# Sota0726/weather-Unet

Measured on AMD Instinct MI355X. Metric: images/sec 256x256 cUNet fwd+bwd, higher is better.
Workload: dtype bf16; 1 GPU; cUNet 256x256 bf16 B=32/GPU, training step: fwd + bwd (dgrad+wgrad) + grad all-reduce + fused Adam; dropout p=0.3 on; random-init weights, 5-class one-hot, loss mean|G(x,c)-x|; global_batch=32, parallelism=dp1

## Files before the change

scratch/stamp_wgrad.py:

```python


def main():
    import sys, os
    sys.path.insert(0, os.path.join(os.path.dirname(__file__), '..', 'weather-unet_amd'))
    import torch
    from wu import _lib, kernels as K
    dev = torch.device('cuda:0'); B = 32
    NWAVES = int(sys.argv[1]) if len(sys.argv) > 1 else 8
    _lib.call('wu_set_option', 2, 1 if NWAVES == 8 else 2)
    dbg = torch.zeros(256 * 8 * 8, dtype=torch.int64, device=dev)
    for name, ci, co, s in [('d1.2', 64, 64, 256), ('d2.2', 128, 128, 128), ('d4.2', 512, 512, 32), ('u1.0', 192, 64, 256), ('u3.0', 768, 256, 64)]:
        x = (torch.rand((B, s, s, ci), device=dev) * 2 - 1).to(torch.bfloat16).permute(0, 3, 1, 2)
        gy = (torch.rand((B, s, s, co), device=dev) * 2 - 1).to(torch.bfloat16).permute(0, 3, 1, 2)
        dw = torch.empty((co, ci, 3, 3), device=dev); db = torch.empty((co,), device=dev)
        for _ in range(20): K.conv3x3_wgrad(x, gy, dw, db)
        torch.cuda.synchronize()
        _lib.call('wu_set_debug_buffer', dbg.data_ptr()); dbg.zero_()
        e0, e1 = torch.cuda.Event(enable_timing=True), torch.cuda.Event(enable_timing=True)
        e0.record(); K.conv3x3_wgrad(x, gy, dw, db); e1.record(); torch.cuda.synchronize()
        _lib.call('wu_set_debug_buffer', None)
        d = dbg.view(256, 8, 8).double().cpu()[:, :NWAVES]
        d = d[d[:, 0, 6] > 0]
        tiles = d[:, 0, 6].mean().item()
        clk = (d[:, 0, 2] / d[:, 0, 3]).median().item() * 0.1
        w, c, tot, bar = d[:, :, 0].mean().item(), d[:, :, 1].mean().item(), d[:, :, 2].mean().item(), d[:, :, 4].mean().item()
        print(f"{name}: wgrad+reduce {e0.elapsed_time(e1)*1e3:.0f} us, tiles/WG {tiles:.1f}; per tile: dma wait {w/tiles:.0f}, barrier {bar/tiles:.0f}, compute {c/tiles:.0f} (ideal 4608); main loop total/tile {tot/tiles:.0f}; in-kernel clock {clk:.2f} GHz")


if __name__ == "__main__":
    main()
```

weather-unet_amd/csrc/conv3x3_wgrad.hip:

```cpp
#include <type_traits>
#include <utility>

#include "wu_common.h"
#include "wgrad_internal.h"

namespace {

template <typename F, int... I> __device__ __forceinline__ void wgrad_static_for_impl(F&& f, std::integer_sequence<int, I...>) {
    (f(std::integral_constant<int, I>{}), ...);
}
template <int N, typename F> __device__ __forceinline__ void wgrad_static_for(F&& f) { wgrad_static_for_impl(f, std::make_integer_sequence<int, N>{}); }

struct WgradArgs {
    const void* x; const void* dy; const void* y;
    float* slab;
    float* bslab;
    int ldx, lddy, ldy;
    int N, H, W, Ho, Wo, Cin, Cout;
    int act;
    int tw_log2, tiles_x, tiles_y, ntiles;
    int splits, co_blocks, ci_blocks;
    int halo_w, halo_h, halo_pix;
};

// ... 275 lines not shown
                const int hp = ry * STRIDE * a.halo_w + rx * STRIDE;
#pragma unroll
                for (int tap = 0; tap < 9; ++tap) {
                    const int kh = tap / 3, kw = tap % 3;
                    const float bv = *(const float*)(x_lds + lds_off<T>(hp + kh * a.halo_w + kw, 0, (32 * wn + l31) * 4));
                    acc[tap] = __builtin_amdgcn_mfma_f32_32x32x2f32(av, bv, acc[tap], 0, 0, 0);
                }
            }
        }
        __syncthreads();
    }

    {
        const int l31 = lane & 31, lh = lane >> 5;
        float* sl = a.slab + (size_t)split * a.Cin;
        const size_t rs = (size_t)a.splits * a.Cin;
#pragma unroll
        for (int tap = 0; tap < 9; ++tap)
#pragma unroll
            for (int i = 0; i < 16; ++i) {
                const int co = cob * 64 + 32 * wm + (i & 3) + 8 * (i >> 2) + 4 * lh;
                const int ci = cib * 64 + 32 * wn + l31;
                sl[((size_t)tap * a.Cout + co) * rs + ci] = acc[tap][i];
            }
    }
    if (cib == 0 && a.bslab) {
        float* red = (float*)smem;
        red[tid] = bsum;
        __syncthreads();
        if (tid < 64) a.bslab[(size_t)split * a.Cout + cob * 64 + tid] = red[tid] + red[tid + 64] + red[tid + 128] + red[tid + 192];
    }
}

__global__ __launch_bounds__(256) __attribute__((amdgpu_num_vgpr(32))) void wgrad_reduce_kernel(
    const float* __restrict__ slab, const float* __restrict__ bslab, float* __restrict__ dw, float* __restrict__ dbias,
    int splits, int Cout, int Cin, int accumulate, int wpr) {
    const int lane = threadIdx.x & 63;
    const int wid = blockIdx.x * 4 + __builtin_amdgcn_readfirstlane((int)(threadIdx.x >> 6));
    const int row = wid / wpr, part = wid - row * wpr;
    if (row >= Cout * 9) return;
    const int co = row / 9, t = row - co * 9;
    const int c4n = (Cin >> 2) / wpr, c4lo = part * c4n;
    int TX = 64;
    while (TX > c4n) TX >>= 1;
    const int G = 64 / TX;
    const int tx = lane & (TX - 1), g = lane / TX;
    const float* base = slab + ((size_t)t * Cout + co) * splits * Cin;
    for (int c4b = 0; c4b < c4n; c4b += TX) {
        const int c4 = c4b + tx;
        const bool valid = c4 < c4n;
        unsigned off = (unsigned)(g * Cin + (c4lo + (valid ? c4 : 0)) * 4);
        const unsigned step = (unsigned)(G * Cin);
        float4 sacc = make_float4(0.f, 0.f, 0.f, 0.f);
        int k = g;
        for (; k + G < splits; k += 2 * G, off += 2 * step) {
            const float4 v0 = *(const float4*)(base + off);
            const float4 v1 = *(const float4*)(base + off + step);
            sacc.x += v0.x; sacc.y += v0.y; sacc.z += v0.z; sacc.w += v0.w;
            sacc.x += v1.x; sacc.y += v1.y; sacc.z += v1.z; sacc.w += v1.w;
        }
        if (k < splits) {
            const float4 v0 = *(const float4*)(base + off);
            sacc.x += v0.x; sacc.y += v0.y; sacc.z += v0.z; sacc.w += v0.w;
        }
        for (int m = TX; m < 64; m <<= 1) {
            sacc.x += __shfl_xor(sacc.x, m); sacc.y += __shfl_xor(sacc.y, m);
            sacc.z += __shfl_xor(sacc.z, m); sacc.w += __shfl_xor(sacc.w, m);
        }
        if (g == 0 && valid) {
            float* o = dw + ((size_t)co * Cin + (c4lo + c4) * 4) * 9 + t;
            if (accumulate) { o[0] += sacc.x; o[9] += sacc.y; o[18] += sacc.z; o[27] += sacc.w; }
            else { o[0] = sacc.x; o[9] = sacc.y; o[18] = sacc.z; o[27] = sacc.w; }
        }
    }
    if (dbias && t == 0 && part == 0) {
        float b = 0.f;
        for (int k = lane; k < splits; k += 64) b += bslab[(size_t)k * Cout + co];
        for (int m = 1; m < 64; m <<= 1) b += __shfl_xor(b, m);
        if (lane == 0) dbias[co] = accumulate ? dbias[co] + b : b;
    }
}

void launch_wgrad_reduce(const float* slab, const float* bslab, float* dw, float* dbias, int splits, int Cout, int Cin, int accumulate, hipStream_t s) {
    int wpr = 1;
    while (wpr < 8 && (long long)splits * (Cin >> 2) > 64LL * 16 * wpr && ((Cin >> 2) % (2 * wpr)) == 0) wpr <<= 1;
    hipLaunchKernelGGL(wgrad_reduce_kernel, dim3(cdiv(Cout * 9 * wpr, 4)), dim3(256), 0, s, slab, bslab, dw, dbias, splits, Cout, Cin, accumulate, wpr);
}

struct WPlan { int P, twl, tiles_x, tiles_y, ntiles, splits, halo_w, halo_h; size_t lds, ws; };

WPlan wgrad_plan(int N, int H, int W, int Cin, int Cout, int stride, int dtype) {
    WPlan p;
    const bool bf = dtype == WU_BF16;
    p.P = bf ? (stride == 1 ? 256 : 128) : (stride == 1 ? 128 : 64);
    const int Ho = (H - 1) / stride + 1, Wo = (W - 1) / stride + 1;
    int twl = 5;
    while (twl > 2 && (1 << (twl - 1)) >= Wo) --twl;
    p.twl = twl;
    const int TW = 1 << twl, TH = p.P >> twl;
    p.tiles_x = cdiv(Wo, TW); p.tiles_y = cdiv(Ho, TH);
    p.ntiles = N * p.tiles_x * p.tiles_y;
    const int blocks = (Cout / 64) * (Cin / 64);
    int splits = cdiv(512, blocks);
    if (splits > p.ntiles) splits = p.ntiles;
    if (splits < 1) splits = 1;
    p.splits = splits;
    p.halo_w = (TW - 1) * stride + 3; p.halo_h = (TH - 1) * stride + 3;
    const int rb = bf ? 128 : 256;
    p.lds = (size_t)(p.P + p.halo_w * p.halo_h) * rb;
    p.ws = ((size_t)splits * 9 * Cout * Cin + (size_t)splits * Cout) * sizeof(float);
    return p;
}

template <typename T, int STRIDE, int P>
void launch_wgrad(const WgradArgs& a, size_t lds, int grid, hipStream_t s) {
    auto kern = conv3x3_wgrad_kernel<T, STRIDE, P>;
    static thread_local bool attr_set = false;
    if (!attr_set) {
        (void)hipFuncSetAttribute((const void*)kern, hipFuncAttributeMaxDynamicSharedMemorySize, 160 * 1024);
// ... 71 lines not shown
```

weather-unet_amd/csrc/conv3x3_wgrad_v2.hip:

```cpp
#include <type_traits>
#include <utility>

#include "wu_common.h"
#include "wgrad_internal.h"

namespace {


struct C {
    static constexpr int P = 256, TH = 8;
    static constexpr int DY_ROW = 128, DY_SLOTS = 8;
    static constexpr int HALO_W = 34, HALO_H = TH + 2, HALO_PIX = HALO_W * HALO_H;
    static constexpr int DY_BYTES = P * DY_ROW;
    static constexpr int DY_PIECES = DY_BYTES / 1024;
    static constexpr int X_PIECES = 48;
    static constexpr int X_BYTES = X_PIECES * 1024;
    static constexpr int BUF = DY_BYTES + X_BYTES;
};

template <int NW_> struct CW {
    static constexpr int NW = NW_;
    static constexpr int NDY = C::DY_PIECES / NW;
    static constexpr int NX = C::X_PIECES / NW;
    static constexpr int PARS = NW == 8 ? 1 : 2;
    static constexpr int NG = 8 * PARS;
};

struct W2Args {
    const bf16_t* x; const bf16_t* dy;
    float* slab; float* bslab;
    unsigned long long* dbg;
    int ldx, lddy;
    int N, H, W, Cin, Cout;
    int tiles_x, tiles_y, ntiles, tiles_per_split, splits, co_blocks, ci_blocks;
    int dma_interleave;
};

__device__ __forceinline__ void dma_wait_all() { asm volatile("s_waitcnt vmcnt(0)" ::: "memory"); }
__device__ __forceinline__ uint4 tr_frag(const char* p0) {
    const s16x4_t a = __builtin_amdgcn_ds_read_tr16_b64_v4i16((s16x4_t __attribute__((address_space(3)))*)p0);
    const s16x4_t b = __builtin_amdgcn_ds_read_tr16_b64_v4i16((s16x4_t __attribute__((address_space(3)))*)(p0 + 4 * 128));
    return make_uint4(((const uint32_t*)&a)[0], ((const uint32_t*)&a)[1], ((const uint32_t*)&b)[0], ((const uint32_t*)&b)[1]);
}
__device__ __forceinline__ void mma(f32x16_t& acc, const uint4& a, const uint4& b) {
    acc = __builtin_amdgcn_mfma_f32_32x32x16_bf16(__builtin_bit_cast(bf16x8_t, a), __builtin_bit_cast(bf16x8_t, b), acc, 0, 0, 0);
}

template <typename F, int... I> __device__ __forceinline__ void static_for_impl(F&& f, std::integer_sequence<int, I...>) {
    (f(std::integral_constant<int, I>{}), ...);
}
template <int N, typename F> __device__ __forceinline__ void static_for(F&& f) { static_for_impl(f, std::make_integer_sequence<int, N>{}); }

template <int HF> __device__ __forceinline__ constexpr int tap_of(int i) { return i == 4 ? 4 : (HF ? 5 + i : i); }

template <int HF, int PARS, typename Issue>
__device__ __forceinline__ void compute_tile(const char* lds, const int (&a_lane)[2], const int (&b_lane)[3], f32x16_t (&acc)[9], Issue&& issue) {
    constexpr int NG = 8 * PARS, NS = 5 * NG;
    auto goff_a = [](int g) { return 32 * (g / PARS) * C::DY_ROW + (g % PARS) * 16 * C::DY_ROW; };
    auto goff_b = [](int g) { return (g / PARS) * C::HALO_W * 128 + (g % PARS) * 16 * 128; };
    auto load_a = [&](int g, int m) __attribute__((always_inline)) { return tr_frag(lds + a_lane[m] + goff_a(g)); };
    auto load_b = [&](int s_) __attribute__((always_inline)) {
        const int g = s_ / 5, i = s_ % 5;
        const int tap = tap_of<HF>(i), kh = tap / 3, kw = tap % 3;
        return tr_frag(lds + b_lane[kw] + goff_b(g) + (kh * C::HALO_W + kw) * 128);
    };
    constexpr int LA = PARS == 1 ? 2 : 5;
    uint4 af[2][2], bf[LA + 1];
    af[0][0] = load_a(0, 0);
// ... 7 lines not shown
        if (PARS == 1) {
            if (i == 0) issue(g);
            if (s_ + LA < NS) bf[(s_ + LA) % (LA + 1)] = load_b(s_ + LA);
            if (g + 1 < NG && i == 1) af[(g + 1) & 1][0] = load_a(g + 1, 0);
            if (g + 1 < NG && i == 2) af[(g + 1) & 1][1] = load_a(g + 1, 1);
            __builtin_amdgcn_sched_barrier(0);
            if constexpr (i < 4) {
                mma(acc[2 * i], af[g & 1][0], b);
                mma(acc[2 * i + 1], af[g & 1][1], b);
            } else {
                mma(acc[8], af[g & 1][HF], b);
            }
            __builtin_amdgcn_sched_barrier(0);
        } else {
            mma(acc[i < 4 ? 2 * i : 8], af[g & 1][i < 4 ? 0 : HF], b);
            if (s_ + LA < NS) bf[(s_ + LA) % (LA + 1)] = load_b(s_ + LA);
            __builtin_amdgcn_sched_barrier(0);
            if constexpr (i < 4) mma(acc[2 * i + 1], af[g & 1][1], b);
            if (g + 1 < NG && i == 1) af[(g + 1) & 1][0] = load_a(g + 1, 0);
            if (g + 1 < NG && i == 2) af[(g + 1) & 1][1] = load_a(g + 1, 1);
            if (i == 0) issue(g);
            __builtin_amdgcn_sched_barrier(0);
        }
    });
}

template <int NW>
__global__ __launch_bounds__(NW * 64) void conv3x3_wgrad_v2_kernel(const W2Args a) {
    using Q = CW<NW>;
    extern __shared__ __attribute__((aligned(16))) char smem[];
    const int tid = threadIdx.x, lane = tid & 63;
    const int wave = __builtin_amdgcn_readfirstlane(tid >> 6);
    const int wci = wave & 1, hf = (wave >> 1) & 1, par = NW == 8 ? wave >> 2 : 0;

    int bid = xcd_remap(blockIdx.x, gridDim.x);
    const int blocks = a.co_blocks * a.ci_blocks;
    const int blk = bid % blocks, split = bid / blocks;
    const int cib = blk % a.ci_blocks, cob = blk / a.ci_blocks;
    const int t_begin = split * a.tiles_per_split;
    const int t_end = min(a.ntiles, t_begin + a.tiles_per_split);

    unsigned dy_off[Q::NDY];
#pragma unroll
    for (int j = 0; j < Q::NDY; ++j) {
        const int i = (NW * j + wave) * 64 + lane;
        const int r = i / C::DY_SLOTS, sl = i % C::DY_SLOTS;
        const int s = sl ^ (((r >> 1) & 1) << 2);
        dy_off[j] = (unsigned)((((r >> 5) * a.W + (r & 31)) * a.lddy + s * 8) * 2);
    }
    unsigned x_off[Q::NX], x_flag[Q::NX];
#pragma unroll
    for (int j = 0; j < Q::NX; ++j) {
        const int i = (NW * j + wave) * 64 + lane;
        const int p = i >> 3, sl = i & 7;
        const int hy = p / C::HALO_W, hx = p - hy * C::HALO_W;
        const int s = sl ^ (((hx >> 1) & 1) << 2);
        x_off[j] = p < C::HALO_PIX ? (unsigned)(((hy * a.W + hx) * a.ldx + s * 8) * 2) : kWuOOB;
        x_flag[j] = (hy == 0 ? 1u : 0u) | (hx == 0 ? 2u : 0u) | (hx == C::HALO_W - 1 ? 4u : 0u);
    }

    const unsigned smem_base = (unsigned)(uintptr_t)(__attribute__((address_space(3))) char*)smem;
    const unsigned dy_img_bytes = (unsigned)((size_t)a.H * a.W * a.lddy * 2);
    const unsigned x_img_bytes = (unsigned)((((size_t)a.H * a.W + a.W) * a.ldx + 64) * 2);
    wu_rsrc_t rs_dy = wu_make_rsrc(a.dy, 0), rs_x = rs_dy;
    unsigned so_dy = 0, so_x = 0, border_f = 0;
    int f_tx = 0, f_ty = 0, f_n = 0;
    {
        int tt = t_begin;
        f_tx = tt % a.tiles_x; tt /= a.tiles_x;
        f_ty = tt % a.tiles_y;
        f_n = tt / a.tiles_y;
    }
    auto set_fetch_tile = [&](bool step) __attribute__((always_inline)) {
        if (step) {
            ++f_tx;
            if (f_tx == a.tiles_x) { f_tx = 0; ++f_ty; }
            if (f_ty == a.tiles_y) { f_ty = 0; ++f_n; }
        }
        const int tx = f_tx, ty = f_ty, n = f_n;
        const int oh0 = ty * C::TH, ow0 = tx * 32;
        rs_dy = wu_make_rsrc(a.dy + (size_t)n * a.H * a.W * a.lddy + cob * 64, dy_img_bytes);
        so_dy = (unsigned)__builtin_amdgcn_readfirstlane((oh0 * a.W + ow0) * a.lddy * 2);
        rs_x = wu_make_rsrc(a.x + ((long long)n * a.H * a.W - (a.W + 1)) * a.ldx + cib * 64, x_img_bytes);
        so_x = (unsigned)__builtin_amdgcn_readfirstlane((oh0 * a.W + ow0) * a.ldx * 2);
        border_f = (unsigned)__builtin_amdgcn_readfirstlane((int)((oh0 == 0 ? 1u : 0u) | (ow0 == 0 ? 2u : 0u) | (ow0 + 32 >= a.W ? 4u : 0u)));
    };
    auto issue_piece = [&](int j, int buf) __attribute__((always_inline)) {
        const unsigned lds = smem_base + buf * C::BUF;
        if (j < Q::NDY) {
            wu_dma16b(dy_off[j], rs_dy, so_dy, __builtin_amdgcn_readfirstlane(lds + (NW * j + wave) * 1024));
        } else {
            const int jj = j - Q::NDY;
            const unsigned vo = (x_flag[jj] & border_f) ? kWuOOB : x_off[jj];
            wu_dma16b(vo, rs_x, so_x, __builtin_amdgcn_readfirstlane(lds + C::DY_BYTES + (NW * jj + wave) * 1024));
        }
    };

    const int g16 = lane >> 4, i16 = lane & 15, q = i16 >> 2, pp = i16 & 3, h = g16 >> 1;
    const int r_lane = 16 * par + 8 * h + q;
    int a_lane[2];
#pragma unroll
    for (int m = 0; m < 2; ++m) {
        const int cb = (32 * m + 16 * (g16 & 1) + 4 * pp) * 2;
        a_lane[m] = r_lane * C::DY_ROW + (cb ^ (((q >> 1) & 1) << 6));
    }
    int b_lane[3];
#pragma unroll
    for (int kw = 0; kw < 3; ++kw) {
        const int cb = (32 * wci + 16 * (g16 & 1) + 4 * pp) * 2;
        b_lane[kw] = C::DY_BYTES + r_lane * 128 + (cb ^ ((((q + kw) >> 1) & 1) << 6));
    }

    f32x16_t acc[9];
#pragma unroll
    for (int t = 0; t < 9; ++t)
#pragma unroll
        for (int i = 0; i < 16; ++i) acc[t][i] = 0.f;
    float bs[8];
#pragma unroll
    for (int e = 0; e < 8; ++e) bs[e] = 0.f;
    const bool do_bias = (cib == 0) && (a.bslab != nullptr);

    unsigned long long t_wait = 0, t_bar = 0, t_comp = 0, t_mark = 0, t_k0 = 0, t_r0 = 0;
#define WU_STAMP(v) do { if (a.dbg) { const unsigned long long t_ = __builtin_readcyclecounter(); v += t_ - t_mark; t_mark = t_; } } while (0)
    if (a.dbg) { t_mark = t_k0 = __builtin_readcyclecounter(); t_r0 = __builtin_amdgcn_s_memrealtime(); }
    auto tile_loop = [&](auto hf_tag) __attribute__((always_inline)) {
        constexpr int HF = decltype(hf_tag)::value;
        if (t_begin < t_end) {
            set_fetch_tile(false);
#pragma unroll
            for (int j = 0; j < Q::NDY + Q::NX; ++j) issue_piece(j, 0);
        }
        for (int tile = t_begin; tile < t_end; ++tile) {
            const int buf = (tile - t_begin) & 1;
            dma_wait_all();
            WU_STAMP(t_wait);
            __syncthreads();
            WU_STAMP(t_bar);
            const bool more = tile + 1 < t_end;
            if (more) set_fetch_tile(true);
            if (more && !a.dma_interleave) {
#pragma unroll
                for (int j = 0; j < Q::NDY + Q::NX; ++j) issue_piece(j, buf ^ 1);
            }
            const char* lds = smem + buf * C::BUF;
            if (do_bias) {
                const int c8 = tid & 7;
#pragma unroll
                for (int r = tid >> 3; r < C::P; r += NW * 8) {
                    const uint4 v = *(const uint4*)(lds + r * C::DY_ROW + ((c8 ^ (((r >> 1) & 1) << 2)) << 4));
                    float f[8];
                    unpack16<bf16_t>(v, f);
#pragma unroll
                    for (int e = 0; e < 8; ++e) bs[e] += f[e];
                }
            }
            compute_tile<HF, Q::PARS>(lds, a_lane, b_lane, acc, [&](int g) __attribute__((always_inline)) {
                if (more && a.dma_interleave && 2 * g < Q::NDY + Q::NX) {
                    issue_piece(2 * g, buf ^ 1);
                    issue_piece(2 * g + 1, buf ^ 1);
                }
            });
            WU_STAMP(t_comp);
        }
    };
    if (hf == 0) tile_loop(std::integral_constant<int, 0>{});
    else tile_loop(std::integral_constant<int, 1>{});
    if (a.dbg && lane == 0) {
        unsigned long long* d = a.dbg + ((size_t)blockIdx.x * 8 + wave) * 8;
        d[0] = t_wait; d[1] = t_comp; d[2] = __builtin_readcyclecounter() - t_k0; d[3] = __builtin_amdgcn_s_memrealtime() - t_r0;
        d[4] = t_bar; d[5] = 0; d[6] = (unsigned long long)(t_end - t_begin); d[7] = 0;
    }
#undef WU_STAMP
    __syncthreads();

    if (NW == 8) {
        float* red = (float*)smem + (size_t)(wave & 3) * 144 * 64;
        if (par == 1) {
#pragma unroll
            for (int t = 0; t < 9; ++t)
#pragma unroll
                for (int i = 0; i < 16; ++i) red[(t * 16 + i) * 64 + lane] = acc[t][i];
        }
        __syncthreads();
        if (par == 0) {
#pragma unroll
            for (int t = 0; t < 9; ++t)
#pragma unroll
                for (int i = 0; i < 16; ++i) acc[t][i] += red[(t * 16 + i) * 64 + lane];
        }
        __syncthreads();
    }

    if (par == 0) {
        const int l31 = lane & 31, lh = lane >> 5;
        float* sl = a.slab + (size_t)split * a.Cin;
        const size_t rs = (size_t)a.splits * a.Cin;
        const int ci = cib * 64 + 32 * wci + l31;
#pragma unroll
        for (int t = 0; t < 9; ++t) {
            const int tap = t == 8 ? 4 : (hf ? 5 + (t >> 1) : (t >> 1));
            const int m = t == 8 ? hf : (t & 1);
#pragma unroll
            for (int i = 0; i < 16; ++i) {
                const int co = cob * 64 + 32 * m + (i & 3) + 8 * (i >> 2) + 4 * lh;
                sl[((size_t)tap * a.Cout + co) * rs + ci] = acc[t][i];
            }
        }
    }
    if (do_bias) {
        float* red = (float*)smem;
#pragma unroll
        for (int e = 0; e < 8; ++e) red[tid * 8 + e] = bs[e];
        __syncthreads();
        if (tid < 64) {
            float s = 0.f;
            for (int j = 0; j < NW * 8; ++j) s += red[(j * 8 + (tid >> 3)) * 8 + (tid & 7)];
            a.bslab[(size_t)split * a.Cout + cob * 64 + tid] = s;
        }
    }
}

}

bool wgrad_v2_eligible(int H, int W, int Cin, int Cout, int stride, int dtype, bool gated) {
    return dtype == WU_BF16 && stride == 1 && !gated && W % 32 == 0 && Cin % 64 == 0 && Cout % 64 == 0;
}

WgradV2Plan wgrad_v2_plan(int N, int H, int W, int Cin, int Cout) {
    WgradV2Plan p;
    p.mode = 0;
    p.tiles_x = cdiv(W, 32); p.tiles_y = cdiv(H, C::TH);
    p.ntiles = N * p.tiles_x * p.tiles_y;
    p.co_blocks = Cout / 64; p.ci_blocks = Cin / 64;
    const int blocks = p.co_blocks * p.ci_blocks;
    int splits = wu_num_cus() / blocks;
    if (splits < 1) splits = 1;
    if (splits > p.ntiles) splits = p.ntiles;
    p.tiles_per_split = cdiv(p.ntiles, splits);
    p.splits = cdiv(p.ntiles, p.tiles_per_split);
    p.ws = ((size_t)p.splits * 9 * Cout * Cin + (size_t)p.splits * Cout) * sizeof(float);
    return p;
}

int wgrad_v2_launch(const void* x, int ldx, const void* dy, int lddy, float* slab, float* bslab,
                    int N, int H, int W, int Cin, int Cout, const WgradV2Plan& p, hipStream_t s) {
    W2Args a;
    a.x = (const bf16_t*)x; a.dy = (const bf16_t*)dy; a.slab = slab; a.bslab = bslab;
    a.ldx = ldx; a.lddy = lddy; a.N = N; a.H = H; a.W = W; a.Cin = Cin; a.Cout = Cout;
    a.tiles_x = p.tiles_x; a.tiles_y = p.tiles_y; a.ntiles = p.ntiles; a.tiles_per_split = p.tiles_per_split;
    a.splits = p.splits; a.co_blocks = p.co_blocks; a.ci_blocks = p.ci_blocks;
    a.dma_interleave = g_wu_opt[WU_OPT_WGRAD_DMA_INTERLEAVE];
    a.dbg = (unsigned long long*)g_wu_dbg_ptr;
    const int grid = p.splits * p.co_blocks * p.ci_blocks;
    static thread_local bool attr_set = false;
    if (!attr_set) {
        (void)hipFuncSetAttribute((const void*)conv3x3_wgrad_v2_kernel<8>, hipFuncAttributeMaxDynamicSharedMemorySize, 160 * 1024);
        (void)hipFuncSetAttribute((const void*)conv3x3_wgrad_v2_kernel<4>, hipFuncAttributeMaxDynamicSharedMemorySize, 160 * 1024);
        attr_set = true;
    }
    if (g_wu_opt[WU_OPT_WGRAD_V2] == 2) hipLaunchKernelGGL(conv3x3_wgrad_v2_kernel<4>, dim3(grid), dim3(256), 2 * C::BUF, s, a);
    else hipLaunchKernelGGL(conv3x3_wgrad_v2_kernel<8>, dim3(grid), dim3(512), 2 * C::BUF, s, a);
    return 0;
}
```

weather-unet_amd/csrc/wu_common.h:

```cpp
#pragma once
#include <hip/hip_runtime.h>
#include <stdint.h>
#include <stdio.h>
#include <string.h>

#include "../../include/wu_kernels.h"

typedef unsigned short bf16_t;
typedef __bf16 bf16x8_t __attribute__((ext_vector_type(8)));
typedef float f32x4_t __attribute__((ext_vector_type(4)));
typedef float f32x16_t __attribute__((ext_vector_type(16)));
typedef short s16x4_t __attribute__((ext_vector_type(4)));

extern thread_local char g_wu_err[256];
#define WU_FAIL(code, ...)                                   \
    do {                                                     \
        snprintf(g_wu_err, sizeof(g_wu_err), __VA_ARGS__);   \
        return (code);                                       \
    } while (0)
#define WU_REQUIRE(cond, ...) \
    do {                      \
        if (!(cond)) WU_FAIL(-1, __VA_ARGS__); \
    } while (0)
#define WU_LAUNCH_CHECK(name)                                                        \
    do {                                                                             \
        hipError_t e_ = hipGetLastError();                                           \
        if (e_ != hipSuccess) WU_FAIL((int)e_, "%s: %s", name, hipGetErrorString(e_)); \
    } while (0)

extern int g_wu_opt[16];
extern void* g_wu_dbg_ptr;
#define WU_OPT_CONV_V2 0
#define WU_OPT_CONV_PERSISTENT 1
#define WU_OPT_WGRAD_V2 2
#define WU_OPT_CONV_SMALL 3
#define WU_OPT_WGRAD_DMA_INTERLEAVE 4
#define WU_OPT_C3_ROWS 5
#define WU_OPT_CONV_PRIO 6
#define WU_OPT_CONV_STRIDED 7
#define WU_OPT_ADAIN_BWD_MARCH 8
#define WU_OPT_ADAIN_FWD_MARCH 9
#define WU_OPT_GRID_CUS 10
#define WU_OPT_CONV_W_RESIDENT 11
#define WU_OPT_PW_TILE 12
#define WU_OPT_IMG3_TILED 13
#define WU_OPT_S2_DGRAD_PARITY 14
#define WU_OPT_PW3 15

int wu_num_cus();

void wu_prof_pre(int family, hipStream_t s);
void wu_prof_post(int family, hipStream_t s, double flops, double bytes);

__device__ __forceinline__ float bf16_to_f32(bf16_t v) { return __uint_as_float(((uint32_t)v) << 16); }
__device__ __forceinline__ bf16_t f32_to_bf16(float f) {
    __bf16 b = (__bf16)f;
    return __builtin_bit_cast(bf16_t, b);
}
__device__ __forceinline__ uint32_t pack_bf16x2(float lo, float hi) {
    typedef float f32x2v __attribute__((ext_vector_type(2)));
    typedef __bf16 bf16x2v __attribute__((ext_vector_type(2)));
    const bf16x2v r = __builtin_convertvector(f32x2v{lo, hi}, bf16x2v);
    return __builtin_bit_cast(uint32_t, r);
}

template <typename T> struct ElemTraits;
template <> struct ElemTraits<float> {
    static constexpr int kPer16B = 4;
    __device__ static __forceinline__ float load(const float* p) { return *p; }
    __device__ static __forceinline__ void store(float* p, float v) { *p = v; }
};
template <> struct ElemTraits<bf16_t> {
    static constexpr int kPer16B = 8;
    __device__ static __forceinline__ float load(const bf16_t* p) { return bf16_to_f32(*p); }
    __device__ static __forceinline__ void store(bf16_t* p, float v) { *p = f32_to_bf16(v); }
};

template <typename T> __device__ __forceinline__ void unpack16(const uint4& v, float* f);
template <> __device__ __forceinline__ void unpack16<float>(const uint4& v, float* f) {
    f[0] = __uint_as_float(v.x); f[1] = __uint_as_float(v.y); f[2] = __uint_as_float(v.z); f[3] = __uint_as_float(v.w);
// ... 76 lines not shown
```

weather-unet_amd/csrc/wu_prof.hip:

```cpp
#include <vector>

#include "wu_common.h"

thread_local char g_wu_err[256] = {0};

extern "C" const char* wu_last_error(void) { return g_wu_err; }
extern "C" int wu_version(void) { return 2; }

int wu_num_cus() {
    if (g_wu_opt[WU_OPT_GRID_CUS] > 0) return g_wu_opt[WU_OPT_GRID_CUS];
    static int cus = 0;
    if (cus == 0) {
        int dev = 0, n = 0;
        if (hipGetDevice(&dev) == hipSuccess && hipDeviceGetAttribute(&n, hipDeviceAttributeMultiprocessorCount, dev) == hipSuccess && n > 0) cus = n;
        else { (void)hipGetLastError(); cus = 256; }
    }
    return cus;
}
extern "C" int wu_cu_count(void) { return wu_num_cus(); }

extern "C" int wu_stream_create_cu_mask(const unsigned* mask, int words, void** stream_out) {
    WU_REQUIRE(mask && words > 0 && stream_out, "stream_create_cu_mask: bad args");
    hipStream_t s = nullptr;
    const hipError_t e = hipExtStreamCreateWithCUMask(&s, (uint32_t)words, mask);
    if (e != hipSuccess) WU_FAIL((int)e, "hipExtStreamCreateWithCUMask: %s", hipGetErrorString(e));
    *stream_out = (void*)s;
    return 0;
}
extern "C" int wu_stream_destroy(void* stream) {
    return hipStreamDestroy((hipStream_t)stream) == hipSuccess ? 0 : -1;
}

extern "C" int wu_event_create(void** event_out) {
    WU_REQUIRE(event_out, "event_create: bad args");
    hipEvent_t e = nullptr;
    const hipError_t rc = hipEventCreateWithFlags(&e, hipEventDisableTiming | hipEventReleaseToDevice);
    if (rc != hipSuccess) WU_FAIL((int)rc, "hipEventCreateWithFlags: %s", hipGetErrorString(rc));
    *event_out = (void*)e;
    return 0;
}
extern "C" int wu_event_destroy(void* event) { return hipEventDestroy((hipEvent_t)event) == hipSuccess ? 0 : -1; }
extern "C" int wu_stream_order_after(void* waiter, void* producer, void* event) {
    WU_REQUIRE(event, "stream_order_after: bad args");
    hipError_t rc = hipEventRecord((hipEvent_t)event, (hipStream_t)producer);
    if (rc == hipSuccess) rc = hipStreamWaitEvent((hipStream_t)waiter, (hipEvent_t)event, 0);
    if (rc != hipSuccess) WU_FAIL((int)rc, "stream_order_after: %s", hipGetErrorString(rc));
    return 0;
}

int g_wu_opt[16] = { 1,  1,  1,  1,  1,  0,  1,  1,  1,  1,  0,  1,  0,  1,  1,  2 + 8 + (128 << 5)};
void* g_wu_dbg_ptr = nullptr;
extern "C" int wu_set_debug_buffer(void* p) { g_wu_dbg_ptr = p; return 0; }
extern "C" int wu_set_option(int key, int value) {
    WU_REQUIRE(key >= 0 && key < 16, "set_option: bad key %d", key);
    g_wu_opt[key] = value;
    return 0;
}

namespace {
constexpr int kMaxFam = 8;
struct Rec { int family; double flops, bytes; };
struct ProfState {
    unsigned mask = 0;
    int used = 0;
    bool open = false;
    std::vector<hipEvent_t> ev;
    std::vector<Rec> rec;
};
ProfState g_prof;
inline bool on(int family) { return g_prof.mask & (1u << family); }
}

void wu_prof_pre(int family, hipStream_t s) {
    if (!g_prof.mask || family <= 0 || family >= kMaxFam || !on(family)) return;
    if ((size_t)(2 * g_prof.used + 2) > g_prof.ev.size()) return;
    (void)hipEventRecord(g_prof.ev[2 * g_prof.used], s);
    g_prof.open = true;
}

void wu_prof_post(int family, hipStream_t s, double flops, double bytes) {
    if (!g_prof.open || !on(family)) return;
    (void)hipEventRecord(g_prof.ev[2 * g_prof.used + 1], s);
    g_prof.rec[g_prof.used] = Rec{family, flops, bytes};
    g_prof.used++;
    g_prof.open = false;
}

// ... 39 lines not shown
```

weather-unet_amd/wu/_lib.py:

```python
import ctypes
import os

from ctypes import c_char_p, c_double, c_float, c_int, c_size_t, c_uint64, c_void_p, POINTER

_PKG = os.path.dirname(os.path.dirname(os.path.abspath(__file__)))
LIB_PATH = os.path.join(_PKG, "lib", "libwu_kernels.so")

F32, BF16 = 0, 1
ACT_NONE, ACT_RELU, ACT_LEAKY = 0, 1, 2
OPT_CONV_V2, OPT_CONV_PERSISTENT, OPT_WGRAD_V2 = 0, 1, 2
FAM_CONV_FWD, FAM_WGRAD, FAM_CONV_DGRAD, FAM_CONV_S2, FAM_WGRAD_S2, FAM_CONV1X1 = 1, 2, 3, 4, 5, 6
FAM_GRID = 7
FAMILY_KERNEL = {1: "conv3x3_mfma_v2_kernel (forward + data-gradient convs; generic conv3x3_mfma_kernel for fp32 / narrow images)",
                 2: "conv3x3_wgrad_v2_kernel (generic conv3x3_wgrad_kernel for fp32 / narrow images)",
                 3: "conv3x3_mfma_kernel<T,1,true> (in-kernel gated dgrad; unused by the fused graph)",
                 4: "stride-2 3x3 conv forward + data gradient: conv1x1_pw3_kernel<.., CONV> (gathered rows); conv3x3_mfma_kernel<T,2,false> / tap-list classes for 64-cout and fp32",
                 5: "conv3x3_wgrad_kernel<T,2>",
                 6: "pointwise convs (estimator): conv1x1_pw3_kernel; conv1x1_mfma_kernel<T> for strided / small / fp32"}

P, I, F, U64, SZ = c_void_p, c_int, c_float, c_uint64, c_size_t

SIGNATURES = {
    "wu_last_error": (c_char_p, []),
    "wu_version": (I, []),
    "wu_cu_count": (I, []),
    "wu_set_option": (I, [I, I]),
    "wu_set_debug_buffer": (I, [P]),
    "wu_stream_create_cu_mask": (I, [P, I, P]),
    "wu_stream_destroy": (I, [P]),
    "wu_spectral_norm_scratch_floats": (SZ, [I, I]),
    "wu_spectral_norm_fwd": (I, [P, I, I, P, P, I, F, P, P, P, P]),
    "wu_spectral_norm_bwd": (I, [P, P, P, P, P, P, I, I, P, P]),
    "wu_event_create": (I, [P]),
    "wu_event_destroy": (I, [P]),
    "wu_stream_order_after": (I, [P, P, P]),
    "wu_spectral_norm_fwd_multi": (I, [I, P, P, P, P, P, I, F, P, P, P, P, P, P]),
    "wu_spectral_norm_bwd_multi": (I, [I, P, P, P, P, P, P, P, P, P, P]),
    "wu_pack_conv3x3": (I, [P, P, P, I, I, P, I, P]),
    "wu_pack_conv3x3_multi": (I, [I, P, P, P, P, P, I, P]),
    "wu_conv3x3_fwd": (I, [P, I, P, P, P, I, I, I, I, I, I, I, I, P, I, I, P, I, I, I, P]),
    "wu_conv3x3_gate_bits_supported": (I, [I, I, I, I, I, I, I]),
    "wu_gate_bits_bytes": (SZ, [I, I, I, I]),
    "wu_conv3x3_fwd_bits": (I, [P, I, P, P, P, I, P, P, I, I, I, I, I, I, I, P]),
# ... 246 lines not shown
```

Measured before the change: 3928 images/sec.

## Split 8-wave wgrad epilogue fold across wave halves and deepen slab reduce

In the 8-wave wgrad v2 kernel, the cross-half accumulator fold is now split so each wave half owns part of the taps. The two halves exchange float4 partials through LDS and store their owned outputs in parallel, instead of half the waves idling while the other half stores everything. The first tile's dy loads are issued before the x-offset setup to hide prologue latency. The split-reduce kernel gains a software-pipelined 4-deep load variant with a lower VGPR cap. Both paths are on by default via a new option (value 3), and debug phase timestamps are added.

```diff
diff --git a/scratch/stamp_wgrad.py b/scratch/stamp_wgrad.py
--- a/scratch/stamp_wgrad.py
+++ b/scratch/stamp_wgrad.py
@@ -7,24 +7,52 @@
     from wu import _lib, kernels as K
     dev = torch.device('cuda:0'); B = 32
     NWAVES = int(sys.argv[1]) if len(sys.argv) > 1 else 8
+    FOLD = int(sys.argv[2]) if len(sys.argv) > 2 else 3
+    REP = int(sys.argv[3]) if len(sys.argv) > 3 else 5
     _lib.call('wu_set_option', 2, 1 if NWAVES == 8 else 2)
+    has_fold = _lib.load().wu_set_option(16, FOLD) == 0
+    print(f"waves {NWAVES}, option 16 = {FOLD if has_fold else 'absent (earlier library)'}")
     dbg = torch.zeros(256 * 8 * 8, dtype=torch.int64, device=dev)
-    for name, ci, co, s in [('d1.2', 64, 64, 256), ('d2.2', 128, 128, 128), ('d4.2', 512, 512, 32), ('u1.0', 192, 64, 256), ('u3.0', 768, 256, 64)]:
+    res = {}
+    layers = [('d2.0', 64, 128, 128), ('d2.2', 128, 128, 128), ('d3.0', 128, 256, 64), ('d3.2', 256, 256, 64),
+              ('d4.0', 256, 512, 32), ('d4.2', 512, 512, 32), ('u1.0', 192, 64, 256), ('d1.2', 64, 64, 256), ('u3.0', 768, 256, 64)]
+    for name, ci, co, s in layers:
         x = (torch.rand((B, s, s, ci), device=dev) * 2 - 1).to(torch.bfloat16).permute(0, 3, 1, 2)
         gy = (torch.rand((B, s, s, co), device=dev) * 2 - 1).to(torch.bfloat16).permute(0, 3, 1, 2)
         dw = torch.empty((co, ci, 3, 3), device=dev); db = torch.empty((co,), device=dev)
         for _ in range(20): K.conv3x3_wgrad(x, gy, dw, db)
         torch.cuda.synchronize()
+        us = []
+        for _ in range(REP):
+            e0, e1 = torch.cuda.Event(enable_timing=True), torch.cuda.Event(enable_timing=True)
+            e0.record()
+            for _ in range(20): K.conv3x3_wgrad(x, gy, dw, db)
+            e1.record(); torch.cuda.synchronize()
+            us.append(e0.elapsed_time(e1) * 1e3 / 20)
+        us.sort()
         _lib.call('wu_set_debug_buffer', dbg.data_ptr()); dbg.zero_()
-        e0, e1 = torch.cuda.Event(enable_timing=True), torch.cuda.Event(enable_timing=True)
-        e0.record(); K.conv3x3_wgrad(x, gy, dw, db); e1.record(); torch.cuda.synchronize()
+        K.conv3x3_wgrad(x, gy, dw, db); torch.cuda.synchronize()
         _lib.call('wu_set_debug_buffer', None)
         d = dbg.view(256, 8, 8).double().cpu()[:, :NWAVES]
         d = d[d[:, 0, 6] > 0]
         tiles = d[:, 0, 6].mean().item()
         clk = (d[:, 0, 2] / d[:, 0, 3]).median().item() * 0.1
         w, c, tot, bar = d[:, :, 0].mean().item(), d[:, :, 1].mean().item(), d[:, :, 2].mean().item(), d[:, :, 4].mean().item()
-        print(f"{name}: wgrad+reduce {e0.elapsed_time(e1)*1e3:.0f} us, tiles/WG {tiles:.1f}; per tile: dma wait {w/tiles:.0f}, barrier {bar/tiles:.0f}, compute {c/tiles:.0f} (ideal 4608); main loop total/tile {tot/tiles:.0f}; in-kernel clock {clk:.2f} GHz")
+        res[name] = (tiles, us[len(us) // 2], us[0], us[-1])
+        line = (f"{name}: wgrad+reduce median {us[len(us) // 2]:.1f} us (min {us[0]:.1f}, max {us[-1]:.1f}), tiles/WG {tiles:.1f}; per tile: dma wait {w/tiles:.0f}, "
+                f"barrier {bar/tiles:.0f}, compute {c/tiles:.0f} (ideal 4608); in-kernel clock {clk:.2f} GHz")
+        if d[:, :, 7].max().item() > 0:
+            pro, loop = d[:, :, 5].mean().item(), (d[:, :, 7] - d[:, :, 5]).mean().item()
+            epi = d[:, :, 2] - d[:, :, 7]
+            k = 1e-3 / clk
+            line += (f"; phases (cycles / us): prologue {pro:.0f} / {pro*k:.2f}, loop {loop:.0f} / {loop*k:.2f}, epilogue mean {epi.mean().item():.0f} / "
+                     f"{epi.mean().item()*k:.2f} max {epi.max().item():.0f} / {epi.max().item()*k:.2f}, kernel {tot:.0f} / {tot*k:.2f}")
+        print(line, flush=True)
+    for a, b in (('d2.0', 'd2.2'), ('d3.0', 'd3.2'), ('d4.0', 'd4.2')):
+        (n1, t1, lo1, hi1), (n2, t2, lo2, hi2) = res[a], res[b]
+        per = (t2 - t1) / (n2 - n1)
+        fixed = [u1 - n1 * (u2 - u1) / (n2 - n1) for u1 in (lo1, hi1) for u2 in (lo2, hi2)]
+        print(f"pair {a} / {b}: {per:.2f} us per tile, fixed per launch {t1 - n1 * per:.1f} us (from the repeats' extremes: {min(fixed):.1f} .. {max(fixed):.1f})", flush=True)
 
 
 if __name__ == "__main__":
diff --git a/weather-unet_amd/csrc/conv3x3_wgrad.hip b/weather-unet_amd/csrc/conv3x3_wgrad.hip
--- a/weather-unet_amd/csrc/conv3x3_wgrad.hip
+++ b/weather-unet_amd/csrc/conv3x3_wgrad.hip
@@ -331,10 +331,11 @@
     }
 }
 
-__global__ __launch_bounds__(256) __attribute__((amdgpu_num_vgpr(32))) void wgrad_reduce_kernel(
+template <bool DEEP>
+__global__ __launch_bounds__(256) __attribute__((amdgpu_num_vgpr(16))) void wgrad_reduce_kernel(
     const float* __restrict__ slab, const float* __restrict__ bslab, float* __restrict__ dw, float* __restrict__ dbias,
     int splits, int Cout, int Cin, int accumulate, int wpr) {
-    const int lane = threadIdx.x & 63;
+    const int lane = (int)__lane_id();
     const int wid = blockIdx.x * 4 + __builtin_amdgcn_readfirstlane((int)(threadIdx.x >> 6));
     const int row = wid / wpr, part = wid - row * wpr;
     if (row >= Cout * 9) return;
@@ -351,16 +352,60 @@
         unsigned off = (unsigned)(g * Cin + (c4lo + (valid ? c4 : 0)) * 4);
         const unsigned step = (unsigned)(G * Cin);
         float4 sacc = make_float4(0.f, 0.f, 0.f, 0.f);
-        int k = g;
-        for (; k + G < splits; k += 2 * G, off += 2 * step) {
-            const float4 v0 = *(const float4*)(base + off);
-            const float4 v1 = *(const float4*)(base + off + step);
-            sacc.x += v0.x; sacc.y += v0.y; sacc.z += v0.z; sacc.w += v0.w;
-            sacc.x += v1.x; sacc.y += v1.y; sacc.z += v1.z; sacc.w += v1.w;
-        }
-        if (k < splits) {
-            const float4 v0 = *(const float4*)(base + off);
-            sacc.x += v0.x; sacc.y += v0.y; sacc.z += v0.z; sacc.w += v0.w;
+        if constexpr (DEEP) {
+            const int n = splits >> __builtin_ctz(G), rem = splits - n * G;
+            const char* const b0 = (const char*)base; const char* const b1 = b0 + 4 * (size_t)step;
+            const char* const b2 = b1 + 4 * (size_t)step; const char* const b3 = b2 + 4 * (size_t)step;
+            unsigned bo = off * 4;
+#define WU_RED_LD(v, j) v = *(const float4*)(b##j + bo)
+#define WU_RED_ADD(v) do { sacc.x += v.x; sacc.y += v.y; sacc.z += v.z; sacc.w += v.w; } while (0)
+            int m = 0;
+            if (n >= 4) {
+                float4 v0, v1, v2, v3;
+                WU_RED_LD(v0, 0); WU_RED_LD(v1, 1); WU_RED_LD(v2, 2); WU_RED_LD(v3, 3);
+                bo += 16 * step;
+                for (m = 4; m + 4 <= n; m += 4, bo += 16 * step) {
+                    WU_RED_ADD(v0); WU_RED_LD(v0, 0); __builtin_amdgcn_sched_barrier(0);
+                    WU_RED_ADD(v1); WU_RED_LD(v1, 1); __builtin_amdgcn_sched_barrier(0);
+                    WU_RED_ADD(v2); WU_RED_LD(v2, 2); __builtin_amdgcn_sched_barrier(0);
+                    WU_RED_ADD(v3); WU_RED_LD(v3, 3); __builtin_amdgcn_sched_barrier(0);
+                }
+                WU_RED_ADD(v0); WU_RED_ADD(v1); WU_RED_ADD(v2); WU_RED_ADD(v3);
+            }
+            if (n - m >= 2) {
+                float4 t0, t1;
+                WU_RED_LD(t0, 0); WU_RED_LD(t1, 1);
+                WU_RED_ADD(t0); WU_RED_ADD(t1);
+                bo += 8 * step;
+            }
+            {
+                const bool more = g < rem;
+                if ((n - m) & 1) {
+                    float4 t0, t1;
+                    WU_RED_LD(t0, 0);
+                    if (more) WU_RED_LD(t1, 1);
+                    WU_RED_ADD(t0);
+                    if (more) WU_RED_ADD(t1);
+                } else if (more) {
+                    float4 t1;
+                    WU_RED_LD(t1, 0);
+                    WU_RED_ADD(t1);
+                }
+            }
+#undef WU_RED_LD
+#undef WU_RED_ADD
+        } else {
+            int k = g;
+            for (; k + G < splits; k += 2 * G, off += 2 * step) {
+                const float4 v0 = *(const float4*)(base + off);
+                const float4 v1 = *(const float4*)(base + off + step);
+                sacc.x += v0.x; sacc.y += v0.y; sacc.z += v0.z; sacc.w += v0.w;
+                sacc.x += v1.x; sacc.y += v1.y; sacc.z += v1.z; sacc.w += v1.w;
+            }
+            if (k < splits) {
+                const float4 v0 = *(const float4*)(base + off);
+                sacc.x += v0.x; sacc.y += v0.y; sacc.z += v0.z; sacc.w += v0.w;
+            }
         }
         for (int m = TX; m < 64; m <<= 1) {
             sacc.x += __shfl_xor(sacc.x, m); sacc.y += __shfl_xor(sacc.y, m);
@@ -383,7 +428,9 @@
 void launch_wgrad_reduce(const float* slab, const float* bslab, float* dw, float* dbias, int splits, int Cout, int Cin, int accumulate, hipStream_t s) {
     int wpr = 1;
     while (wpr < 8 && (long long)splits * (Cin >> 2) > 64LL * 16 * wpr && ((Cin >> 2) % (2 * wpr)) == 0) wpr <<= 1;
-    hipLaunchKernelGGL(wgrad_reduce_kernel, dim3(cdiv(Cout * 9 * wpr, 4)), dim3(256), 0, s, slab, bslab, dw, dbias, splits, Cout, Cin, accumulate, wpr);
+    const dim3 grid(cdiv(Cout * 9 * wpr, 4));
+    if (g_wu_opt[WU_OPT_WGRAD_FOLD] & 2) hipLaunchKernelGGL(wgrad_reduce_kernel<true>, grid, dim3(256), 0, s, slab, bslab, dw, dbias, splits, Cout, Cin, accumulate, wpr);
+    else hipLaunchKernelGGL(wgrad_reduce_kernel<false>, grid, dim3(256), 0, s, slab, bslab, dw, dbias, splits, Cout, Cin, accumulate, wpr);
 }
 
 struct WPlan { int P, twl, tiles_x, tiles_y, ntiles, splits, halo_w, halo_h; size_t lds, ws; };
diff --git a/weather-unet_amd/csrc/conv3x3_wgrad_v2.hip b/weather-unet_amd/csrc/conv3x3_wgrad_v2.hip
--- a/weather-unet_amd/csrc/conv3x3_wgrad_v2.hip
+++ b/weather-unet_amd/csrc/conv3x3_wgrad_v2.hip
@@ -34,6 +34,7 @@
     int N, H, W, Cin, Cout;
     int tiles_x, tiles_y, ntiles, tiles_per_split, splits, co_blocks, ci_blocks;
     int dma_interleave;
+    int fold8;
 };
 
 __device__ __forceinline__ void dma_wait_all() { asm volatile("s_waitcnt vmcnt(0)" ::: "memory"); }
@@ -107,6 +108,8 @@
     const int tid = threadIdx.x, lane = tid & 63;
     const int wave = __builtin_amdgcn_readfirstlane(tid >> 6);
     const int wci = wave & 1, hf = (wave >> 1) & 1, par = NW == 8 ? wave >> 2 : 0;
+    unsigned long long t_k0 = 0, t_r0 = 0, t_pro = 0, t_loop = 0;
+    if (a.dbg) { t_k0 = __builtin_readcyclecounter(); t_r0 = __builtin_amdgcn_s_memrealtime(); }
 
     int bid = xcd_remap(blockIdx.x, gridDim.x);
     const int blocks = a.co_blocks * a.ci_blocks;
@@ -124,15 +127,6 @@
         dy_off[j] = (unsigned)((((r >> 5) * a.W + (r & 31)) * a.lddy + s * 8) * 2);
     }
     unsigned x_off[Q::NX], x_flag[Q::NX];
-#pragma unroll
-    for (int j = 0; j < Q::NX; ++j) {
-        const int i = (NW * j + wave) * 64 + lane;
-        const int p = i >> 3, sl = i & 7;
-        const int hy = p / C::HALO_W, hx = p - hy * C::HALO_W;
-        const int s = sl ^ (((hx >> 1) & 1) << 2);
-        x_off[j] = p < C::HALO_PIX ? (unsigned)(((hy * a.W + hx) * a.ldx + s * 8) * 2) : kWuOOB;
-        x_flag[j] = (hy == 0 ? 1u : 0u) | (hx == 0 ? 2u : 0u) | (hx == C::HALO_W - 1 ? 4u : 0u);
-    }
 
     const unsigned smem_base = (unsigned)(uintptr_t)(__attribute__((address_space(3))) char*)smem;
     const unsigned dy_img_bytes = (unsigned)((size_t)a.H * a.W * a.lddy * 2);
@@ -171,6 +165,26 @@
         }
     };
 
+    if (t_begin < t_end) {
+        set_fetch_tile(false);
+#pragma unroll
+        for (int j = 0; j < Q::NDY; ++j) issue_piece(j, 0);
+    }
+    __builtin_amdgcn_sched_barrier(0);
+#pragma unroll
+    for (int j = 0; j < Q::NX; ++j) {
+        const int i = (NW * j + wave) * 64 + lane;
+        const int p = i >> 3, sl = i & 7;
+        const int hy = p / C::HALO_W, hx = p - hy * C::HALO_W;
+        const int s = sl ^ (((hx >> 1) & 1) << 2);
+        x_off[j] = p < C::HALO_PIX ? (unsigned)(((hy * a.W + hx) * a.ldx + s * 8) * 2) : kWuOOB;
+        x_flag[j] = (hy == 0 ? 1u : 0u) | (hx == 0 ? 2u : 0u) | (hx == C::HALO_W - 1 ? 4u : 0u);
+    }
+    if (t_begin < t_end) {
+#pragma unroll
+        for (int j = Q::NDY; j < Q::NDY + Q::NX; ++j) issue_piece(j, 0);
+    }
+
     const int g16 = lane >> 4, i16 = lane & 15, q = i16 >> 2, pp = i16 & 3, h = g16 >> 1;
     const int r_lane = 16 * par + 8 * h + q;
     int a_lane[2];
@@ -196,22 +210,18 @@
     for (int e = 0; e < 8; ++e) bs[e] = 0.f;
     const bool do_bias = (cib == 0) && (a.bslab != nullptr);
 
-    unsigned long long t_wait = 0, t_bar = 0, t_comp = 0, t_mark = 0, t_k0 = 0, t_r0 = 0;
+    unsigned long long t_wait = 0, t_bar = 0, t_comp = 0, t_mark = 0;
 #define WU_STAMP(v) do { if (a.dbg) { const unsigned long long t_ = __builtin_readcyclecounter(); v += t_ - t_mark; t_mark = t_; } } while (0)
-    if (a.dbg) { t_mark = t_k0 = __builtin_readcyclecounter(); t_r0 = __builtin_amdgcn_s_memrealtime(); }
+    if (a.dbg) t_mark = __builtin_readcyclecounter();
     auto tile_loop = [&](auto hf_tag) __attribute__((always_inline)) {
         constexpr int HF = decltype(hf_tag)::value;
-        if (t_begin < t_end) {
-            set_fetch_tile(false);
-#pragma unroll
-            for (int j = 0; j < Q::NDY + Q::NX; ++j) issue_piece(j, 0);
-        }
         for (int tile = t_begin; tile < t_end; ++tile) {
             const int buf = (tile - t_begin) & 1;
             dma_wait_all();
             WU_STAMP(t_wait);
             __syncthreads();
             WU_STAMP(t_bar);
+            if (a.dbg && tile == t_begin) t_pro = t_mark - t_k0;
             const bool more = tile + 1 < t_end;
             if (more) set_fetch_tile(true);
             if (more && !a.dma_interleave) {
@@ -241,57 +251,98 @@
     };
     if (hf == 0) tile_loop(std::integral_constant<int, 0>{});
     else tile_loop(std::integral_constant<int, 1>{});
-    if (a.dbg && lane == 0) {
-        unsigned long long* d = a.dbg + ((size_t)blockIdx.x * 8 + wave) * 8;
-        d[0] = t_wait; d[1] = t_comp; d[2] = __builtin_readcyclecounter() - t_k0; d[3] = __builtin_amdgcn_s_memrealtime() - t_r0;
-        d[4] = t_bar; d[5] = 0; d[6] = (unsigned long long)(t_end - t_begin); d[7] = 0;
-    }
+    if (a.dbg) t_loop = __builtin_readcyclecounter() - t_k0;
 #undef WU_STAMP
     __syncthreads();
 
-    if (NW == 8) {
-        float* red = (float*)smem + (size_t)(wave & 3) * 144 * 64;
-        if (par == 1) {
+    float* const sl = a.slab + (size_t)split * a.Cin;
+    const size_t rs = (size_t)a.splits * a.Cin;
+    const int l31 = lane & 31, lh = lane >> 5;
+    const int ci = cib * 64 + 32 * wci + l31;
+    auto store_acc = [&](int t, int i, float v) __attribute__((always_inline)) {
+        const int tap = t == 8 ? 4 : (hf ? 5 + (t >> 1) : (t >> 1));
+        const int m = t == 8 ? hf : (t & 1);
+        const int co = cob * 64 + 32 * m + (i & 3) + 8 * (i >> 2) + 4 * lh;
+        sl[((size_t)tap * a.Cout + co) * rs + ci] = v;
+    };
+    float* const bred = (float*)(smem + 144 * 1024);
+
+    if (NW == 8 && a.fold8) {
+        float4* const ex = (float4*)smem + (size_t)(wave & 3) * 36 * 64;
+        auto own = [](int t, int i) { return t < 4 ? 0 : (t < 8 ? 1 : (i < 8 ? 0 : 1)); };
+        auto slot = [](int t, int i) { return t == 8 ? 16 + ((i & 7) >> 2) : 4 * (t & 3) + (i >> 2); };
+        auto fold = [&](auto par_tag) __attribute__((always_inline)) {
+            constexpr int PAR = decltype(par_tag)::value;
 #pragma unroll
             for (int t = 0; t < 9; ++t)
 #pragma unroll
-                for (int i = 0; i < 16; ++i) red[(t * 16 + i) * 64 + lane] = acc[t][i];
-        }
-        __syncthreads();
+                for (int i = 0; i < 16; i += 4)
+                    if (own(t, i) != PAR) ex[((1 - PAR) * 18 + slot(t, i)) * 64 + lane] = make_float4(acc[t][i], acc[t][i + 1], acc[t][i + 2], acc[t][i + 3]);
+            if (do_bias) {
+                *(float4*)(bred + tid * 8) = make_float4(bs[0], bs[1], bs[2], bs[3]);
+                *(float4*)(bred + tid * 8 + 4) = make_float4(bs[4], bs[5], bs[6], bs[7]);
+            }
+            __syncthreads();
+#pragma unroll
+            for (int t = 0; t < 9; ++t)
+#pragma unroll
+                for (int i = 0; i < 16; i += 4)
+                    if (own(t, i) == PAR) {
+                        const float4 o = ex[(PAR * 18 + slot(t, i)) * 64 + lane];
+                        store_acc(t, i, acc[t][i] + o.x); store_acc(t, i + 1, acc[t][i + 1] + o.y);
+                        store_acc(t, i + 2, acc[t][i + 2] + o.z); store_acc(t, i + 3, acc[t][i + 3] + o.w);
+                    }
+        };
+        if (par == 0) fold(std::integral_constant<int, 0>{});
+        else fold(std::integral_constant<int, 1>{});
+        if (do_bias && tid < 64) {
+            float s = 0.f;
+            for (int j = 0; j < NW * 8; ++j) s += bred[(j * 8 + (tid >> 3)) * 8 + (tid & 7)];
+            a.bslab[(size_t)split * a.Cout + cob * 64 + tid] = s;
+        }
+    } else {
+        if (NW == 8) {
+            float* red = (float*)smem + (size_t)(wave & 3) * 144 * 64;
+            if (par == 1) {
+#pragma unroll
+                for (int t = 0; t < 9; ++t)
+#pragma unroll
+                    for (int i = 0; i < 16; ++i) red[(t * 16 + i) * 64 + lane] = acc[t][i];
+            }
+            __syncthreads();
+            if (par == 0) {
+#pragma unroll
+                for (int t = 0; t < 9; ++t)
+#pragma unroll
+                    for (int i = 0; i < 16; ++i) acc[t][i] += red[(t * 16 + i) * 64 + lane];
+            }
+            __syncthreads();
+        }
+
         if (par == 0) {
 #pragma unroll
             for (int t = 0; t < 9; ++t)
 #pragma unroll
-                for (int i = 0; i < 16; ++i) acc[t][i] += red[(t * 16 + i) * 64 + lane];
-        }
-        __syncthreads();
-    }
-
-    if (par == 0) {
-        const int l31 = lane & 31, lh = lane >> 5;
-        float* sl = a.slab + (size_t)split * a.Cin;
-        const size_t rs = (size_t)a.splits * a.Cin;
-        const int ci = cib * 64 + 32 * wci + l31;
-#pragma unroll
-        for (int t = 0; t < 9; ++t) {
-            const int tap = t == 8 ? 4 : (hf ? 5 + (t >> 1) : (t >> 1));
-            const int m = t == 8 ? hf : (t & 1);
-#pragma unroll
-            for (int i = 0; i < 16; ++i) {
-                const int co = cob * 64 + 32 * m + (i & 3) + 8 * (i >> 2) + 4 * lh;
-                sl[((size_t)tap * a.Cout + co) * rs + ci] = acc[t][i];
-            }
-        }
-    }
-    if (do_bias) {
-        float* red = (float*)smem;
-#pragma unroll
-        for (int e = 0; e < 8; ++e) red[tid * 8 + e] = bs[e];
-        __syncthreads();
-        if (tid < 64) {
-            float s = 0.f;
-            for (int j = 0; j < NW * 8; ++j) s += red[(j * 8 + (tid >> 3)) * 8 + (tid & 7)];
-            a.bslab[(size_t)split * a.Cout + cob * 64 + tid] = s;
+                for (int i = 0; i < 16; ++i) store_acc(t, i, acc[t][i]);
+        }
+        if (do_bias) {
+            float* red = (float*)smem;
+#pragma unroll
+            for (int e = 0; e < 8; ++e) red[tid * 8 + e] = bs[e];
+            __syncthreads();
+            if (tid < 64) {
+                float s = 0.f;
+                for (int j = 0; j < NW * 8; ++j) s += red[(j * 8 + (tid >> 3)) * 8 + (tid & 7)];
+                a.bslab[(size_t)split * a.Cout + cob * 64 + tid] = s;
+            }
+        }
+    }
+    if (a.dbg) {
+        asm volatile("s_waitcnt vmcnt(0)" ::: "memory");
+        if (lane == 0) {
+            unsigned long long* d = a.dbg + ((size_t)blockIdx.x * 8 + wave) * 8;
+            d[0] = t_wait; d[1] = t_comp; d[2] = __builtin_readcyclecounter() - t_k0; d[3] = __builtin_amdgcn_s_memrealtime() - t_r0;
+            d[4] = t_bar; d[5] = t_pro; d[6] = (unsigned long long)(t_end - t_begin); d[7] = t_loop;
         }
     }
 }
@@ -326,6 +377,7 @@
     a.tiles_x = p.tiles_x; a.tiles_y = p.tiles_y; a.ntiles = p.ntiles; a.tiles_per_split = p.tiles_per_split;
     a.splits = p.splits; a.co_blocks = p.co_blocks; a.ci_blocks = p.ci_blocks;
     a.dma_interleave = g_wu_opt[WU_OPT_WGRAD_DMA_INTERLEAVE];
+    a.fold8 = g_wu_opt[WU_OPT_WGRAD_FOLD] & 1;
     a.dbg = (unsigned long long*)g_wu_dbg_ptr;
     const int grid = p.splits * p.co_blocks * p.ci_blocks;
     static thread_local bool attr_set = false;
diff --git a/weather-unet_amd/csrc/wu_common.h b/weather-unet_amd/csrc/wu_common.h
--- a/weather-unet_amd/csrc/wu_common.h
+++ b/weather-unet_amd/csrc/wu_common.h
@@ -28,7 +28,8 @@
         if (e_ != hipSuccess) WU_FAIL((int)e_, "%s: %s", name, hipGetErrorString(e_)); \
     } while (0)
 
-extern int g_wu_opt[16];
+#define WU_OPT_COUNT 17
+extern int g_wu_opt[WU_OPT_COUNT];
 extern void* g_wu_dbg_ptr;
 #define WU_OPT_CONV_V2 0
 #define WU_OPT_CONV_PERSISTENT 1
@@ -46,6 +47,7 @@
 #define WU_OPT_IMG3_TILED 13
 #define WU_OPT_S2_DGRAD_PARITY 14
 #define WU_OPT_PW3 15
+#define WU_OPT_WGRAD_FOLD 16
 
 int wu_num_cus();
 
diff --git a/weather-unet_amd/csrc/wu_prof.hip b/weather-unet_amd/csrc/wu_prof.hip
--- a/weather-unet_amd/csrc/wu_prof.hip
+++ b/weather-unet_amd/csrc/wu_prof.hip
@@ -48,11 +48,11 @@
     return 0;
 }
 
-int g_wu_opt[16] = { 1,  1,  1,  1,  1,  0,  1,  1,  1,  1,  0,  1,  0,  1,  1,  2 + 8 + (128 << 5)};
+int g_wu_opt[WU_OPT_COUNT] = { 1,  1,  1,  1,  1,  0,  1,  1,  1,  1,  0,  1,  0,  1,  1,  2 + 8 + (128 << 5),  3};
 void* g_wu_dbg_ptr = nullptr;
 extern "C" int wu_set_debug_buffer(void* p) { g_wu_dbg_ptr = p; return 0; }
 extern "C" int wu_set_option(int key, int value) {
-    WU_REQUIRE(key >= 0 && key < 16, "set_option: bad key %d", key);
+    WU_REQUIRE(key >= 0 && key < WU_OPT_COUNT, "set_option: bad key %d", key);
     g_wu_opt[key] = value;
     return 0;
 }
diff --git a/weather-unet_amd/wu/_lib.py b/weather-unet_amd/wu/_lib.py
--- a/weather-unet_amd/wu/_lib.py
+++ b/weather-unet_amd/wu/_lib.py
@@ -9,6 +9,7 @@
 F32, BF16 = 0, 1
 ACT_NONE, ACT_RELU, ACT_LEAKY = 0, 1, 2
 OPT_CONV_V2, OPT_CONV_PERSISTENT, OPT_WGRAD_V2 = 0, 1, 2
+OPT_WGRAD_FOLD = 16
 FAM_CONV_FWD, FAM_WGRAD, FAM_CONV_DGRAD, FAM_CONV_S2, FAM_WGRAD_S2, FAM_CONV1X1 = 1, 2, 3, 4, 5, 6
 FAM_GRID = 7
 FAMILY_KERNEL = {1: "conv3x3_mfma_v2_kernel (forward + data-gradient convs; generic conv3x3_mfma_kernel for fp32 / narrow images)",
```

Result: no change. 3954 images/sec (median of 6 runs) (+0.7%).
